# caidao22/pnode

Measured on AMD Instinct MI355X. Metric: time-steps/sec (fwd+adjoint), higher is better.
Workload: dtype f32; 1 GPU; C3a: MLP dynamics 3x512 tanh, batch 4096 x state_dim 512 per GPU, rk4 fixed h=0.01, 100 time steps, adjoint on, stages stored in HBM; batch_per_gpu=4096, state_elements_per_gpu=2097152, rejected_attempts=0, launch_mode=graph(auto), graph_revalidate_every=100, linear_param_grads=engine (8 of 8 parameter tensors; fused dW + db MFMA kernel on 4 layers), stage_tapes_retained=True, tunableop=False, parallelism=batch-sharded x1, one RCCL all-reduce of dL/dtheta per backward

## Files before the change

include/pnode_amd.h:

```cpp
#ifndef PNODE_AMD_H
#define PNODE_AMD_H

#include <stdint.h>

#ifdef __cplusplus
extern "C" {
#endif

#define PN_MAX_STAGES 7
#define PN_MAX_TERMS 8
#define PN_WGRAD_MAX_PAIRS 8
#define PN_WGRAD_EXACT_FP32 1
#define PN_WGRAD_TILE_64 2
#define PN_ABI_VERSION 4

typedef enum { PN_F32 = 0, PN_F64 = 1 } pn_dtype;

const char *pn_last_error(void);
int pn_abi_version(void);

typedef struct {
  int s;
  int order;
  int fsal;
// ... 46 lines not shown
int pn_colsum_accum_multi(void *stream, int dtype, int nsrc, const int64_t *rows, const int64_t *cols, const void *const *g,
                          void *const *mu, const double *alpha, void *work);
int64_t pn_colsum_work_bytes(int nsrc, const int64_t *rows, const int64_t *cols);
int pn_colsum_accum(void *stream, int dtype, int64_t rows, int64_t cols, const void *g, void *mu, double alpha, void *work);

typedef struct {
  const void *g, *x;
  void *pw, *pb;
  double alpha;
  int64_t out_f, in_f;
} pn_wgrad_pair;
int pn_linear_wgrad_supported(int dtype, int64_t rows, int64_t out_f, int64_t in_f);
int64_t pn_linear_wgrad_work_bytes(int dtype, int64_t out_f, int64_t in_f, int64_t *bias_bytes);
int pn_linear_wgrad(void *stream, int dtype, int64_t rows, int64_t out_f, int64_t in_f, const void *g, const void *x, double alpha,
                    void *pw, void *pb);
int pn_linear_wgrad_group(void *stream, int dtype, int64_t rows, int npairs, const pn_wgrad_pair *pairs, int flags);
int pn_linear_wgrad_finish(void *stream, int dtype, int64_t out_f, int64_t in_f, void *pw, void *pb, void *mu_w, void *mu_b);

#define PN_ACT_IDENTITY 0
#define PN_ACT_TANH 1
int pn_linear_fwd_supported(int dtype, int64_t rows, int64_t out_f, int64_t in_f);
int pn_linear_fwd(void *stream, int dtype, int64_t rows, int64_t out_f, int64_t in_f, const void *x, const void *w, const void *b, int act,
                  void *y);

int pn_linear_bwd_supported(int dtype, int64_t rows, int64_t out_f, int64_t in_f);
int pn_linear_bwd(void *stream, int dtype, int64_t rows, int64_t out_f, int64_t in_f, const void *g, const void *a, const void *w, void *gz,
                  void *dx);

int pn_dots(void *stream, int dtype, int64_t n, const void *x, int nk, const void *const *y,
            void *work, double *result_dev);
int64_t pn_dots_work_bytes(int64_t n);
int pn_lincomb(void *stream, int dtype, int64_t n, void *out, int nin, const void *const *x, const double *c);
int pn_stream_wait_scalars(void *stream, const double *host_ptr, int count, double *values);

int pn_copy(void *stream, int dtype, int64_t n, void *y, const void *x);
int pn_zero(void *stream, int dtype, int64_t n, void *y);

typedef enum { PN_K_STAGE = 0, PN_K_COMBINE_WRMS, PN_K_ADJ_THETA, PN_K_ADJ_ACCUM,
               PN_K_PARAM_ACCUM, PN_K_COPY, PN_K_DOTS, PN_K_LINCOMB, PN_K_LINEAR_WGRAD, PN_K_COUNT } pn_kernel_id;
int pn_prof_enable(int on);
int pn_prof_is_enabled(void);
int pn_tune_set(const char *spec);
int pn_prof_collect(int count, int64_t *launches, double *usec, double *bytes);
const char *pn_kernel_name(int kernel_id);

typedef struct pn_ts pn_ts;

pn_ts *pn_ts_create(void);
void pn_ts_destroy(pn_ts *ts);
int pn_ts_set_rk_type(pn_ts *ts, const char *rk_type);
// ... 160 lines not shown
```

pnode_amd/_lib.py:

```python
import ctypes
import os

import torch

_HERE = os.path.dirname(os.path.abspath(__file__))
LIB_PATH = os.path.join(_HERE, "lib", "libpnode_amd.so")

PN_MAX_STAGES = 7
PN_MAX_TERMS = 8
PN_F32, PN_F64 = 0, 1
PN_TRAJ_ALL, PN_TRAJ_SOLUTION, PN_TRAJ_BUDGET = 0, 1, 2
KERNEL_IDS = ("pn_rk_stage", "pn_rk_combine_wrms", "pn_adj_theta", "pn_adj_accum", "pn_param_accum", "pn_copy", "pn_dots", "pn_lincomb",
              "pn_linear_wgrad")


class PnError(RuntimeError):
    """A C-ABI entry point returned non-zero (stands where petsc4py.PETSc.Error did)."""


class Tableau(ctypes.Structure):
    _fields_ = [
        ("s", ctypes.c_int), ("order", ctypes.c_int), ("fsal", ctypes.c_int), ("has_embed", ctypes.c_int),
        ("A", (ctypes.c_double * PN_MAX_STAGES) * PN_MAX_STAGES),
        ("b", ctypes.c_double * PN_MAX_STAGES),
        ("bembed", ctypes.c_double * PN_MAX_STAGES),
        ("c", ctypes.c_double * PN_MAX_STAGES),
    ]


class WgradPair(ctypes.Structure):
    _fields_ = [("g", ctypes.c_void_p), ("x", ctypes.c_void_p), ("pw", ctypes.c_void_p), ("pb", ctypes.c_void_p),
                ("alpha", ctypes.c_double), ("out_f", ctypes.c_int64), ("in_f", ctypes.c_int64)]


PN_WGRAD_MAX_PAIRS = 8
PN_WGRAD_EXACT_FP32 = 1
PN_WGRAD_TILE_64 = 2
PN_ACT_IDENTITY, PN_ACT_TANH = 0, 1
PN_ABI_VERSION = 4
PN_DENSE_MAX_POW = 4
PN_DENSE_CHUNK = 32
PN_DENSE_NONTEMPORAL = 1
PN_ROWS_T, PN_ROWS_H, PN_ROWS_TFIRST, PN_ROWS_CACHED, PN_ROWS_ND = 0, 1, 2, 3, 4
PN_ROWS_SPANCTR, PN_ROWS_STEPS, PN_ROWS_REJ, PN_ROWS_REJ_STEP, PN_ROWS_PREV_REJ, PN_ROWS_FINISHED, PN_ROWS_FAIL, PN_ROWS_NI = 0, 1, 2, 3, 4, 5, 6, 8
_vp, _i, _i64, _d, _cp = ctypes.c_void_p, ctypes.c_int, ctypes.c_int64, ctypes.c_double, ctypes.c_char_p
_pd, _pi, _pi64 = ctypes.POINTER(ctypes.c_double), ctypes.POINTER(ctypes.c_int), ctypes.POINTER(ctypes.c_int64)
_pvp = ctypes.POINTER(ctypes.c_void_p)

STAGE_CB = ctypes.CFUNCTYPE(ctypes.c_int64, ctypes.c_void_p, ctypes.c_int, ctypes.c_double)
VJP_CB = ctypes.CFUNCTYPE(ctypes.c_int64, ctypes.c_void_p, ctypes.c_int, ctypes.c_double, ctypes.c_int, ctypes.c_double)
RK_STAGE_FN = ctypes.CFUNCTYPE(_i, _vp, _i, _i64, _vp, _vp, _i, _pvp, _pd)
RK_COMBINE_WRMS_FN = ctypes.CFUNCTYPE(_i, _vp, _i, _i64, _vp, _vp, _i, _pvp, _pd, _pd, _d, _d, _vp, _vp)
ADJ_THETA_FN = ctypes.CFUNCTYPE(_i, _vp, _i, _i64, _vp, _vp, _d, _i, _pvp, _pd)
ADJ_ACCUM_FN = ctypes.CFUNCTYPE(_i, _vp, _i, _i64, _vp, _vp, _i, _pvp, _pd, _vp, _vp, _d)


class VecOps(ctypes.Structure):
    _fields_ = [("rk_stage", RK_STAGE_FN), ("rk_combine_wrms", RK_COMBINE_WRMS_FN), ("adj_theta", ADJ_THETA_FN),
                ("adj_accum", ADJ_ACCUM_FN)]


# ... 46 lines not shown
    "pn_stream_wait_winf": (_i, [_vp, _vp, _i64, _pd]),
    "pn_winf_finish": (_i, [_vp, _i64, _pd]),
    "pn_pinned_scalar": (_i, [ctypes.POINTER(_vp), ctypes.POINTER(_vp)]),
    "pn_pinned_free": (_i, [_vp]),
    "pn_stream_create": (_i, [_i, ctypes.POINTER(_vp)]),
    "pn_stream_destroy": (_i, [_vp]),
    "pn_pinned_block": (_i, [_i64, ctypes.POINTER(_vp), ctypes.POINTER(_vp)]),
    "pn_stream_wait_scalar": (_i, [_vp, _vp, _pd]),
    "pn_adj_theta": (_i, [_vp, _i, _i64, _vp, _vp, _d, _i, _pvp, _pd]),
    "pn_adj_accum": (_i, [_vp, _i, _i64, _vp, _vp, _i, _pvp, _pd, _vp, _vp, _d]),
    "pn_param_accum": (_i, [_vp, _i, _vp, _d, _i, _pvp, _pi64, _pi64]),
    "pn_param_accum_multi": (_i, [_vp, _i, _vp, _i, _pd, _i, _pvp, _pi64, _pi64]),
    "pn_lincomb": (_i, [_vp, _i, _i64, _vp, _i, _pvp, _pd]),
    "pn_dots": (_i, [_vp, _i, _i64, _vp, _i, _pvp, _vp, _vp]),
    "pn_dots_work_bytes": (_i64, [_i64]),
    "pn_stream_wait_scalars": (_i, [_vp, _vp, _i, _pd]),
    "pn_linear_wgrad_supported": (_i, [_i, _i64, _i64, _i64]),
    "pn_linear_wgrad_work_bytes": (_i64, [_i, _i64, _i64, _pi64]),
    "pn_linear_wgrad": (_i, [_vp, _i, _i64, _i64, _i64, _vp, _vp, _d, _vp, _vp]),
    "pn_linear_wgrad_group": (_i, [_vp, _i, _i64, _i, ctypes.POINTER(WgradPair), _i]),
    "pn_linear_wgrad_finish": (_i, [_vp, _i, _i64, _i64, _vp, _vp, _vp, _vp]),
    "pn_linear_fwd_supported": (_i, [_i, _i64, _i64, _i64]),
    "pn_linear_fwd": (_i, [_vp, _i, _i64, _i64, _i64, _vp, _vp, _vp, _i, _vp]),
    "pn_linear_bwd_supported": (_i, [_i, _i64, _i64, _i64]),
    "pn_linear_bwd": (_i, [_vp, _i, _i64, _i64, _i64, _vp, _vp, _vp, _vp, _vp]),
    "pn_colsum_accum": (_i, [_vp, _i, _i64, _i64, _vp, _vp, _d, _vp]),
    "pn_colsum_accum_multi": (_i, [_vp, _i, _i, _pi64, _pi64, ctypes.POINTER(_vp), ctypes.POINTER(_vp), _pd, _vp]),
    "pn_colsum_work_bytes": (_i64, [_i, _pi64, _pi64]),
    "pn_copy": (_i, [_vp, _i, _i64, _vp, _vp]),
    "pn_zero": (_i, [_vp, _i, _i64, _vp]),
    "pn_prof_enable": (_i, [_i]),
    "pn_prof_is_enabled": (_i, []),
    "pn_tune_set": (_i, [_cp]),
    "pn_prof_collect": (_i, [_i, _pi64, _pd, _pd]),
    "pn_kernel_name": (_cp, [_i]),
    "pn_ts_create": (_vp, []),
    "pn_ts_destroy": (None, [_vp]),
    "pn_ts_set_rk_type": (_i, [_vp, _cp]),
    "pn_ts_get_tableau": (_i, [_vp, ctypes.POINTER(Tableau)]),
    "pn_ts_set_option": (_i, [_vp, _cp, _cp]),
    "pn_ts_wnorm_infinity": (_i, [_vp]),
    "pn_ts_is_adaptive": (_i, [_vp]),
    "pn_ts_set_scheme": (_i, [_vp, _i, _i]),
    "pn_ts_get_tolerances": (_i, [_vp, _pd, _pd]),
    "pn_ts_begin": (_i, [_vp, _d, _d, _i, _pd]),
    "pn_ts_attempt": (_i, [_vp, _pd, _pd]),
    "pn_ts_judge": (_i, [_vp, _d, _pi, _pi, _pi]),
    "pn_ts_count_fixed_steps": (_i64, [_vp]),
# ... 91 lines not shown
```

pnode_amd/_rk_sweep.py:

```python
import contextlib
import ctypes
import warnings

import torch

from . import _lib, options
from ._lib import PnError, check


def _mem_now(device):
    try:
        st = torch._C._cuda_memoryStats(device.index if device.index is not None else torch.cuda.current_device())
        return st["allocated_bytes"]["all"]["current"], st["reserved_bytes"]["all"]["current"]
    except Exception:
        return torch.cuda.memory_allocated(device), torch.cuda.memory_reserved(device)


class _RKState(object):
    __slots__ = "save T times full solution sol traj keep_tape tape_budget tape_steps tape_fsal K_fsal pingpong pp cur cur_slot ctl finished".split()


class RKSweep(object):
    def _func_with_grad(self, t, y, which="EX"):
        fn, params, names = ((self.funcIM, self._paramsI, self._pnamesI) if which == "IM"
# ... 694 lines not shown
            self._ops.wgrad_flags = (_lib.PN_WGRAD_EXACT_FP32 if exact else 0) | (_lib.PN_WGRAD_TILE_64 if tile64 else 0)
        self._setup_linear_fwd()
        sig = (id(self.funcEX), on, self._stepper_kind in (None, "imex"), tuple(id(p) for p in self._paramsE), gemm, side_on, exact, tile64)
        if sig == self._lin_sig:
            return
        self._lin_sig = sig
        if self._lin is not None:
            self._lin.remove()
            self._lin = None
        if on and sig[2] and self._paramsE:
            from ._lineargrad import LinearParamGrads
            lin = LinearParamGrads(self)
            lin.fused = not gemm
            lin.side_on = side_on
            lin.side_priority = side != "same-priority"
            if lin.install(self.funcEX, self._paramsE, self._poffE if self._stepper_kind == "imex" else self._poff):
                self._lin = lin

    def _setup_linear_fwd(self):
        mode = str(options.get_all().get("pn_linear_fwd", "auto"))
        mode = "auto" if mode == "auto" else ("1" if options.truthy(mode, False) else "0")
        bwd = str(options.get_all().get("pn_linear_bwd", "auto"))
        bwd = "auto" if bwd == "auto" else ("1" if options.truthy(bwd, False) else "0")
        from ._linearfwd import LinearFwd
        on = mode != "0" and self._stepper_kind in (None, "imex") and self.device.type == LinearFwd.device_type \
            and self.tensor_dtype == torch.float32 and hasattr(self._ops, "linear_fwd")
        sig = (id(self.funcEX), mode, on, tuple(id(p) for p in self._paramsE), bwd)
        if sig == self._fwd_sig:
            return
        self._fwd_sig = sig
        self._fwd = None
        if on and self._paramsE:
            fwd = LinearFwd(self)
            if fwd.install(self.funcEX, self._paramsE, mode, bwd):
                self._fwd = fwd

    @property
    def linear_fwd(self):
        fwd = self._fwd
        if fwd is None:
            return "stock modules (no eligible pair, not an fp32 state on a HIP device, a theta stepper, or -pn_linear_fwd 0)"
        if fwd.disabled:
            return "stock modules (%s)" % fwd.why
        return "fused (%d pairs, %d calls so far)" % (sum(len(p) for _, p in fwd.plans), fwd.n_fused)

    @property
    def linear_bwd(self):
        fwd = self._fwd
        if fwd is None or fwd.disabled:
            return "torch operations (the pairs run the stock modules: see linear_fwd)"
# ... 256 lines not shown
```

pnode_amd/_vecops.py:

```python
import contextlib
import ctypes
import warnings

import torch
import torch.nn as nn

from . import _lib, options
from ._lib import PnError, check


class HipVecOps(object):

    def __init__(self, device, dtype, n):
        if device.type != "cuda":
            raise RuntimeError(
                "pnode_amd runs on MI355X HIP devices only (got a %s tensor); there is no CPU path" % device.type)
        self.lib = _lib.load()
        self.device, self.dtype, self.n = device, dtype, n
        self.code = _lib.dtype_code(dtype)
        self.work = None
        self.dots_work = None
        self._err_host = self._err_dev = None
        self._pinned_stream = None
        self._seg_cache = {}
# ... 151 lines not shown
        self.linear_wgrad_group([(g, x, alpha, pw, pb)])

    MAX_WGRAD_PAIRS = _lib.PN_WGRAD_MAX_PAIRS

    wgrad_flags = 0

    def linear_wgrad_group(self, items, stream=None):
        st = self.stream() if stream is None else stream
        for k in range(0, len(items), self.MAX_WGRAD_PAIRS):
            part = items[k:k + self.MAX_WGRAD_PAIRS]
            arr = (_lib.WgradPair * len(part))()
            for q, (g, x, alpha, pw, pb) in zip(arr, part):
                q.g, q.x, q.pw, q.pb = g.data_ptr(), x.data_ptr(), pw.data_ptr(), (None if pb is None else pb.data_ptr())
                q.alpha, q.out_f, q.in_f = alpha, g.shape[1], x.shape[1]
            check(self.lib.pn_linear_wgrad_group(st, self.code, part[0][0].shape[0], len(part), arr, self.wgrad_flags))

    def linear_wgrad_finish(self, out_f, in_f, pw, pb, mu_w, mu_b):
        check(self.lib.pn_linear_wgrad_finish(self.stream(), self.code, out_f, in_f, pw.data_ptr(), None if pb is None else pb.data_ptr(),
                                              mu_w.data_ptr(), None if mu_b is None else mu_b.data_ptr()))

    def linear_fwd_supported(self, rows, out_f, in_f):
        return bool(self.lib.pn_linear_fwd_supported(self.code, rows, out_f, in_f))

    def linear_fwd(self, x, w, b, tanh, y=None):
        rows, in_f = x.shape
        out_f = w.shape[0]
        for v in (x, w, b, y):
            if v is not None and not (v.is_contiguous() and v.dtype == torch.float32 and v.device == x.device and x.is_cuda):
                raise PnError("pn_linear_fwd: contiguous fp32 tensors on one HIP device")
        if w.shape[1] != in_f or (b is not None and b.numel() != out_f):
            raise PnError("pn_linear_fwd: x (rows, in_f), w (out_f, in_f), b (out_f,)")
        if y is None:
            y = torch.empty((rows, out_f), dtype=x.dtype, device=x.device)
        elif tuple(y.shape) != (rows, out_f):
            raise PnError("pn_linear_fwd: y (rows, out_f)")
        check(self.lib.pn_linear_fwd(self.stream(), _lib.dtype_code(x.dtype), rows, out_f, in_f, x.data_ptr(), w.data_ptr(),
                                     None if b is None else b.data_ptr(), _lib.PN_ACT_TANH if tanh else _lib.PN_ACT_IDENTITY, y.data_ptr()))
        return y

    def linear_bwd_supported(self, rows, out_f, in_f):
        return bool(self.lib.pn_linear_bwd_supported(self.code, rows, out_f, in_f))

    def linear_bwd(self, g, a, w, gz=None, dx=None):
        rows, out_f = g.shape
        in_f = w.shape[1]
        for v in (g, a, w, gz, dx):
            if v is not None and not (v.is_contiguous() and v.dtype == torch.float32 and v.device == g.device and g.is_cuda):
                raise PnError("pn_linear_bwd: contiguous fp32 tensors on one HIP device")
        if tuple(a.shape) != (rows, out_f) or w.shape[0] != out_f:
            raise PnError("pn_linear_bwd: g and a (rows, out_f), w (out_f, in_f)")
        if gz is None:
            gz = torch.empty((rows, out_f), dtype=g.dtype, device=g.device)
        elif tuple(gz.shape) != (rows, out_f):
            raise PnError("pn_linear_bwd: gz (rows, out_f)")
        if dx is None:
            dx = torch.empty((rows, in_f), dtype=g.dtype, device=g.device)
        elif tuple(dx.shape) != (rows, in_f):
            raise PnError("pn_linear_bwd: dx (rows, in_f)")
        check(self.lib.pn_linear_bwd(self.stream(), self.code, rows, out_f, in_f, g.data_ptr(), a.data_ptr(), w.data_ptr(), gz.data_ptr(),
                                     dx.data_ptr()))
        return gz, dx

    dense_flags = _lib.PN_DENSE_NONTEMPORAL

    def dense_eval(self, out, u, Ks, coefs):
        m, nk = len(coefs), len(Ks)
        c = (ctypes.c_double * (m * nk))(*[x for row in coefs for x in row])
        check(self.lib.pn_rk_dense_eval(self.stream(), self.code, self.n, u.data_ptr(), nk, (ctypes.c_void_p * nk)(*[k.data_ptr() for k in Ks]),
                                        m, c, out.data_ptr(), out.stride(0), self.dense_flags))

    def dense_adjoint(self, Ds, G, g, coefs, accumulate=False):
        m, nd = g.shape[0], len(Ds)
        c = (ctypes.c_double * max(m * nd, 1))(*[x for row in coefs for x in row])
        check(self.lib.pn_rk_dense_adjoint(self.stream(), self.code, self.n, m, g.data_ptr(), g.stride(0), nd, c,
                                           (ctypes.c_void_p * max(nd, 1))(*[d.data_ptr() for d in Ds]),
                                           None if G is None else G.data_ptr(), 1 if accumulate else 0))

    def _tgrad_work(self):
        w = getattr(self, "_tg_work", None)
        if w is None:
            w = self._tg_work = torch.zeros(self.lib.pn_tgrad_work_bytes(self.n) // 8, dtype=torch.float64, device=self.device)
        return w

# ... 214 lines not shown
```

pnode_amd/csrc/pn_linear.hip:

```cpp
#include <hip/hip_runtime.h>

#include <cstdint>
#include <string>
#include <type_traits>

#include "pn_launch.h"
#include "pnode_amd.h"

namespace {

typedef float f32x16 __attribute__((ext_vector_type(16)));
typedef float f32x4 __attribute__((ext_vector_type(4)));
typedef double f64x4 __attribute__((ext_vector_type(4)));
typedef double f64x2 __attribute__((ext_vector_type(2)));

constexpr int kSplit = 8;
constexpr int BM = 64, BN = 64;
constexpr int kThreads = 512;
constexpr int kMaxPairs = PN_WGRAD_MAX_PAIRS;
constexpr int64_t kMaxWeights = (int64_t)1 << 22;

template <typename T>
struct Shape {
  static constexpr int BK = 32;
// ... 519 lines not shown
  for (int e = 0; e < VEC; ++e) z[e] = (T)0;
#pragma unroll
  for (int s = 0; s < kSplit; ++s) *reinterpret_cast<vec_t *>(PW + (size_t)s * mn + i) = z;
}

template <typename T>
__global__ __launch_bounds__(256) void pn_linear_bgrad_finish_kernel(double *__restrict__ PB, int M, int parts, T *__restrict__ mu) {
  const int m = blockIdx.x * 256 + threadIdx.x;
  if (m >= M) return;
  double s = 0.0;
  int k = 0;
  for (; k + 8 <= parts; k += 8) {
    double v[8];
#pragma unroll
    for (int j = 0; j < 8; ++j) v[j] = PB[(size_t)(k + j) * M + m];
#pragma unroll
    for (int j = 0; j < 8; ++j) s += v[j];
  }
  for (; k < parts; ++k) s += PB[(size_t)k * M + m];
  mu[m] += (T)s;
  for (k = 0; k < parts; ++k) PB[(size_t)k * M + m] = 0.0;
}

constexpr int FM = 64, FN = 128, FK = 32, kFwdThreads = 512;

struct FwdArgs {
  const float *x, *w, *b;
  float *y;
  int rows, out_f, in_f, act, ntn;
};

template <bool RAGGED>
__device__ __forceinline__ void linear_fwd_body(const FwdArgs &a) {
  constexpr int ROWB = 2 * FK, XPART = FM * ROWB, WPART = FN * ROWB, BUF = 3 * XPART + 3 * WPART;
  __shared__ __attribute__((aligned(16))) char smem[2 * BUF];
  const float *__restrict__ X = a.x;
  const float *__restrict__ W = a.w;
  const int rows = a.rows, out_f = a.out_f, in_f = a.in_f, ntn = a.ntn;
  const int nblk = (int)gridDim.x, bid = (int)blockIdx.x;
  const int tile = nblk % 8 == 0 ? (bid & 7) * (nblk >> 3) + (bid >> 3) : bid;
  const int tm = tile / ntn, tn = tile % ntn;
  const int t = threadIdx.x, lane = t & 63, w = t >> 6;
  const int kh = w >> 2, wm = w & 1, wn = (w >> 1) & 1;
  const int lrow = t >> 3, lc = t & 7;
  const int nslab = in_f / FK;
  const bool xok = !RAGGED || tm * FM + lrow < rows;
  const bool wok0 = !RAGGED || tn * FN + lrow < out_f, wok1 = !RAGGED || tn * FN + 64 + lrow < out_f;
  const float *xp = X + (size_t)(tm * FM + lrow) * in_f + lc * 4;
  const float *wp0 = W + (size_t)(tn * FN + lrow) * in_f + lc * 4;
  const float *wp1 = wp0 + (size_t)64 * in_f;
  const f32x4 zero4 = {0.f, 0.f, 0.f, 0.f};
  f32x4 xv, wv0, wv1;
  f32x16 acc0, acc1;
#pragma unroll
  for (int e = 0; e < 16; ++e) acc0[e] = 0.f, acc1[e] = 0.f;

  auto gload = [&](int slab) {
    xv = xok ? *reinterpret_cast<const f32x4 *>(xp + slab * FK) : zero4;
// ... 10 lines not shown
  auto lstore = [&](int buf) {
    char *b = smem + buf * BUF;
    split_store(xv, b, XPART);
    split_store(wv0, b + 3 * XPART, WPART);
    split_store(wv1, b + 3 * XPART + 64 * ROWB, WPART);
  };
  auto frag = [&](const char *part, int r0) -> s16x8 {
    const int row = r0 + (lane & 31);
    return *reinterpret_cast<const s16x8 *>(part + row * ROWB + (swz_row(row, 2 * kh + (lane >> 5)) << 4));
  };
  auto compute = [&](int buf) {
    const char *xb = smem + buf * BUF, *wb = xb + 3 * XPART;
    const s16x8 ah = frag(xb, wm * 32), am = frag(xb + XPART, wm * 32), al = frag(xb + 2 * XPART, wm * 32);
    {
      const s16x8 bh = frag(wb, wn * 64), bm = frag(wb + WPART, wn * 64), bl = frag(wb + 2 * WPART, wn * 64);
      six_products(acc0, ah, am, al, bh, bm, bl);
    }
    {
      const s16x8 bh = frag(wb, wn * 64 + 32), bm = frag(wb + WPART, wn * 64 + 32), bl = frag(wb + 2 * WPART, wn * 64 + 32);
      six_products(acc1, ah, am, al, bh, bm, bl);
    }
  };

  gload(0);
  lstore(0);
  if (nslab > 1) gload(1);
  __syncthreads();
  for (int s = 0; s < nslab; ++s) {
    if (s + 1 < nslab) lstore((s + 1) & 1);
    compute(s & 1);
    if (s + 2 < nslab) gload(s + 2);
    __syncthreads();
  }
  float(*red)[64] = reinterpret_cast<float(*)[64]>(smem);
  static_assert(sizeof(smem) >= 8 * 16 * 64 * sizeof(float), "the exchange is staged in the slab buffers");
#pragma unroll
  for (int e = 0; e < 16; ++e) red[w * 16 + e][lane] = kh == 0 ? acc1[e] : acc0[e];
  __syncthreads();
  const int col = tn * FN + wn * 64 + kh * 32 + (lane & 31);
  const bool colok = !RAGGED || col < out_f;
  const float bias = (a.b != nullptr && colok) ? a.b[col] : 0.f;
  const int row0 = tm * FM + wm * 32 + 4 * (lane >> 5);
  float *yp = a.y + (size_t)row0 * out_f + col;
  const bool tanh_act = a.act == PN_ACT_TANH;
#pragma unroll
  for (int e = 0; e < 16; ++e) {
    const float other = red[(w ^ 4) * 16 + e][lane];
    const float first = kh == 0 ? acc0[e] : other, second = kh == 0 ? other : acc1[e];
    float z = (first + second) + bias;
    if (tanh_act) z = tanhf(z);
    const int r = (e & 3) + 8 * (e >> 2);
    if (colok && (!RAGGED || row0 + r < rows)) yp[(size_t)r * out_f] = z;
  }
}

__global__ __launch_bounds__(kFwdThreads, 4) void pn_linear_fwd_kernel_f32x3(FwdArgs a) { linear_fwd_body<false>(a); }
__global__ __launch_bounds__(kFwdThreads, 4) void pn_linear_fwd_kernel_f32x3_ragged(FwdArgs a) { linear_fwd_body<true>(a); }

struct BwdArgs {
  const float *g, *a, *w;
  float *gz, *dx;
  int rows, out_f, in_f, ntn;
};

template <bool RAGGED>
__device__ __forceinline__ void linear_bwd_body(const BwdArgs &q) {
  constexpr int AROWB = 2 * FK, APART = FM * AROWB;
  constexpr int WROWB = 128, WIMG = FK * WROWB, WPART = 2 * WIMG;
  constexpr int BUF = 3 * APART + 3 * WPART;
  __shared__ __attribute__((aligned(16))) char smem[2 * BUF];
  const float *__restrict__ G = q.g;
  const float *__restrict__ A = q.a;
  const float *__restrict__ W = q.w;
  const int rows = q.rows, out_f = q.out_f, in_f = q.in_f, ntn = q.ntn;
  const int nblk = (int)gridDim.x, bid = (int)blockIdx.x;
  const int tile = nblk % 8 == 0 ? (bid & 7) * (nblk >> 3) + (bid >> 3) : bid;
  const int tm = tile / ntn, tn = tile % ntn;
  const int t = threadIdx.x, lane = t & 63, w = t >> 6;
  const int kh = w >> 2, wm = w & 1, wn = (w >> 1) & 1;
  const int lrow = t >> 3, lc = t & 7;
  const int krow = t >> 5, sub = (t >> 4) & 1, kc = t & 15;
  const int nslab = out_f / FK;
  const bool aok = !RAGGED || tm * FM + lrow < rows;
  const bool wok = !RAGGED || tn * FN + sub * 64 + kc * 4 < in_f;
  const bool keep = tn == 0 && aok;
  const size_t aoff = (size_t)(tm * FM + lrow) * out_f + lc * 4;
  const float *wp = W + (size_t)krow * in_f + tn * FN + sub * 64 + kc * 4;
  const f32x4 zero4 = {0.f, 0.f, 0.f, 0.f};
  f32x4 gv, av, wv0, wv1;
  f32x16 acc0, acc1;
#pragma unroll
  for (int e = 0; e < 16; ++e) acc0[e] = 0.f, acc1[e] = 0.f;

// ... 30 lines not shown
    s16x4 r[2];
#pragma unroll
    for (int u = 0; u < 2; ++u) {
      const int k = kh * 16 + 8 * (g4 >> 1) + 4 * u + q4;
      const int c = col0 + (g4 & 1) * 16 + 4 * p4;
      r[u] = __builtin_amdgcn_ds_read_tr16_b64_v4i16((__attribute__((address_space(3))) s16x4 *)(img + k * WROWB + swz_tr(k, c) * 2));
    }
    const s16x8 f = {r[0][0], r[0][1], r[0][2], r[0][3], r[1][0], r[1][1], r[1][2], r[1][3]};
    return f;
  };
  auto compute = [&](int buf) {
    const char *ab = smem + buf * BUF, *wb = ab + 3 * APART + wn * WIMG;
    const s16x8 ah = afrag(ab, wm * 32), am = afrag(ab + APART, wm * 32), al = afrag(ab + 2 * APART, wm * 32);
    {
      const s16x8 bh = wfrag(wb, 0), bm = wfrag(wb + WPART, 0), bl = wfrag(wb + 2 * WPART, 0);
      six_products(acc0, ah, am, al, bh, bm, bl);
    }
    {
      const s16x8 bh = wfrag(wb, 32), bm = wfrag(wb + WPART, 32), bl = wfrag(wb + 2 * WPART, 32);
      six_products(acc1, ah, am, al, bh, bm, bl);
    }
  };

  gload(0);
  lstore(0, 0);
  if (nslab > 1) gload(1);
  __syncthreads();
  for (int s = 0; s < nslab; ++s) {
    if (s + 1 < nslab) lstore(s + 1, (s + 1) & 1);
    compute(s & 1);
    if (s + 2 < nslab) gload(s + 2);
    __syncthreads();
  }
  float(*red)[64] = reinterpret_cast<float(*)[64]>(smem);
  static_assert(sizeof(smem) >= 8 * 16 * 64 * sizeof(float), "the exchange is staged in the slab buffers");
#pragma unroll
  for (int e = 0; e < 16; ++e) red[w * 16 + e][lane] = kh == 0 ? acc1[e] : acc0[e];
  __syncthreads();
  const int col = tn * FN + wn * 64 + kh * 32 + (lane & 31);
  const bool colok = !RAGGED || col < in_f;
  const int row0 = tm * FM + wm * 32 + 4 * (lane >> 5);
  float *dp = q.dx + (size_t)row0 * in_f + col;
#pragma unroll
  for (int e = 0; e < 16; ++e) {
    const float other = red[(w ^ 4) * 16 + e][lane];
    const float first = kh == 0 ? acc0[e] : other, second = kh == 0 ? other : acc1[e];
    const int r = (e & 3) + 8 * (e >> 2);
    if (colok && (!RAGGED || row0 + r < rows)) dp[(size_t)r * in_f] = first + second;
  }
}

__global__ __launch_bounds__(kFwdThreads, 4) void pn_linear_bwd_kernel_f32x3(BwdArgs a) { linear_bwd_body<false>(a); }
__global__ __launch_bounds__(kFwdThreads, 4) void pn_linear_bwd_kernel_f32x3_ragged(BwdArgs a) { linear_bwd_body<true>(a); }

int cu_count() {
  static int n = 0;
  if (n == 0) {
    int dev = 0, v = 0;
    if (hipGetDevice(&dev) == hipSuccess && hipDeviceGetAttribute(&v, hipDeviceAttributeMultiprocessorCount, dev) == hipSuccess && v > 0)
      n = v;
    else
      n = 256;
  }
  return n;
}

template <typename T>
int finish_t(hipStream_t st, int64_t out_f, int64_t in_f, void *pw, void *pb, void *mu_w, void *mu_b) {
  const size_t mn = (size_t)out_f * (size_t)in_f;
  constexpr int VEC = 16 / (int)sizeof(T);
  const char *name = "pn_linear_wgrad_finish";
  int rc = pn::launch(name, pn_linear_wgrad_finish_kernel<T>, dim3((unsigned)((mn / VEC + 255) / 256)), dim3(256), st, (T *)pw, mn, (T *)mu_w);
  if (!rc && pb != nullptr && mu_b != nullptr)
    rc = pn::launch(name, pn_linear_bgrad_finish_kernel<T>, dim3((unsigned)((out_f + 255) / 256)), dim3(256), st, (double *)pb, (int)out_f,
                    (int)(kSplit * (in_f / BN)), (T *)mu_b);
  return rc;
// ... 62 lines not shown

int pn_linear_wgrad(void *stream, int dtype, int64_t rows, int64_t out_f, int64_t in_f, const void *g, const void *x, double alpha,
                    void *pw, void *pb) {
  pn_wgrad_pair q;
  q.g = g, q.x = x, q.pw = pw, q.pb = pb, q.alpha = alpha, q.out_f = out_f, q.in_f = in_f;
  return pn_linear_wgrad_group(stream, dtype, rows, 1, &q, 0);
}

int pn_linear_wgrad_finish(void *stream, int dtype, int64_t out_f, int64_t in_f, void *pw, void *pb, void *mu_w, void *mu_b) {
  if (dtype != PN_F32 && dtype != PN_F64) return pn::fail("pn_linear_wgrad_finish: fp32 or fp64");
  if (!pn::aligned16(pw, mu_w)) return pn::fail("pn_linear_wgrad_finish: operands must be 16-byte aligned");
  return pn::with_dtype(dtype, [&](auto t) { return finish_t<decltype(t)>((hipStream_t)stream, out_f, in_f, pw, pb, mu_w, mu_b); });
}

int pn_linear_fwd_supported(int dtype, int64_t rows, int64_t out_f, int64_t in_f) {
  if (dtype != PN_F32) return 0;
  const int64_t lim = (int64_t)1 << 30;
  if (!(rows >= 256 && rows < lim && out_f > 0 && out_f < lim && out_f % 64 == 0 && in_f > 0 && in_f < lim && in_f % 64 == 0)) return 0;
  return ((rows + FM - 1) / FM) * ((out_f + FN - 1) / FN) < lim ? 1 : 0;
}

int pn_linear_fwd(void *stream, int dtype, int64_t rows, int64_t out_f, int64_t in_f, const void *x, const void *w, const void *b, int act,
                  void *y) {
  if (!pn_linear_fwd_supported(dtype, rows, out_f, in_f)) return pn::fail("pn_linear_fwd: unsupported dtype or shape (see pn_linear_fwd_supported)");
  if (act != PN_ACT_IDENTITY && act != PN_ACT_TANH) return pn::fail("pn_linear_fwd: act is PN_ACT_IDENTITY or PN_ACT_TANH");
  if (x == nullptr || w == nullptr || y == nullptr) return pn::fail("pn_linear_fwd: null operand");
  if (!pn::aligned16(x, w, y) || (reinterpret_cast<uintptr_t>(b) & 3)) return pn::fail("pn_linear_fwd: operands must be 16-byte aligned");
  if (x == y) return pn::fail("pn_linear_fwd: y must not be x (other workgroups still read the rows a workgroup writes)");
  FwdArgs a;
  a.x = (const float *)x, a.w = (const float *)w, a.b = (const float *)b, a.y = (float *)y;
  a.rows = (int)rows, a.out_f = (int)out_f, a.in_f = (int)in_f, a.act = act;
  a.ntn = (int)((out_f + FN - 1) / FN);
  const unsigned blocks = (unsigned)((rows + FM - 1) / FM) * (unsigned)a.ntn;
  const bool ragged = rows % FM != 0 || out_f % FN != 0;
  return pn::launch("pn_linear_fwd", ragged ? pn_linear_fwd_kernel_f32x3_ragged : pn_linear_fwd_kernel_f32x3, dim3(blocks), dim3(kFwdThreads),
                    (hipStream_t)stream, a);
}

int pn_linear_bwd_supported(int dtype, int64_t rows, int64_t out_f, int64_t in_f) {
  if (dtype != PN_F32) return 0;
  const int64_t lim = (int64_t)1 << 30;
  if (!(rows >= 256 && rows < lim && out_f > 0 && out_f < lim && out_f % 64 == 0 && in_f > 0 && in_f < lim && in_f % 64 == 0)) return 0;
  return ((rows + FM - 1) / FM) * ((in_f + FN - 1) / FN) < lim ? 1 : 0;
}

int pn_linear_bwd(void *stream, int dtype, int64_t rows, int64_t out_f, int64_t in_f, const void *g, const void *a, const void *w, void *gz,
                  void *dx) {
  if (!pn_linear_bwd_supported(dtype, rows, out_f, in_f)) return pn::fail("pn_linear_bwd: unsupported dtype or shape (see pn_linear_bwd_supported)");
  if (g == nullptr || a == nullptr || w == nullptr || gz == nullptr || dx == nullptr) return pn::fail("pn_linear_bwd: null operand");
  if (!pn::aligned16(g, a, w, gz, dx)) return pn::fail("pn_linear_bwd: operands must be 16-byte aligned");
  const size_t nz = (size_t)rows * (size_t)out_f * sizeof(float), nw = (size_t)out_f * (size_t)in_f * sizeof(float),
               nx = (size_t)rows * (size_t)in_f * sizeof(float);
  auto overlap = [](const void *p, size_t np, const void *r, size_t nr) {
    const uintptr_t p0 = reinterpret_cast<uintptr_t>(p), r0 = reinterpret_cast<uintptr_t>(r);
    return p0 < r0 + nr && r0 < p0 + np;
  };
  if (overlap(gz, nz, g, nz) || overlap(gz, nz, a, nz) || overlap(gz, nz, w, nw))
    return pn::fail("pn_linear_bwd: gz must not alias g, a or w (other workgroups still read them)");
  if (overlap(dx, nx, g, nz) || overlap(dx, nx, a, nz) || overlap(dx, nx, w, nw) || overlap(dx, nx, gz, nz))
    return pn::fail("pn_linear_bwd: dx must not alias g, a, w or gz");
  BwdArgs q;
  q.g = (const float *)g, q.a = (const float *)a, q.w = (const float *)w, q.gz = (float *)gz, q.dx = (float *)dx;
  q.rows = (int)rows, q.out_f = (int)out_f, q.in_f = (int)in_f;
  q.ntn = (int)((in_f + FN - 1) / FN);
  const unsigned blocks = (unsigned)((rows + FM - 1) / FM) * (unsigned)q.ntn;
  const bool ragged = rows % FM != 0 || in_f % FN != 0;
  return pn::launch("pn_linear_bwd", ragged ? pn_linear_bwd_kernel_f32x3_ragged : pn_linear_bwd_kernel_f32x3, dim3(blocks), dim3(kFwdThreads),
                    (hipStream_t)stream, q);
}

}
```

pnode_amd/options.py:

```python
import os
import shlex

_DB = {}


def _is_key(tok):
    if not tok.startswith("-") or len(tok) < 2:
        return False
    try:
        float(tok)
        return False
    except ValueError:
        return True


def parse(argv):
    out = {}
    toks = list(argv)
    i = 0
    while i < len(toks):
        tok = toks[i]
        if _is_key(tok):
            key = tok.lstrip("-")
            if i + 1 < len(toks) and not _is_key(toks[i + 1]):
# ... 20 lines not shown
def set_option(key, value=""):
    _DB[key.lstrip("-")] = "" if value is None else str(value)


def del_option(key):
    _DB.pop(key.lstrip("-"), None)


def clear():
    _DB.clear()


def get_all():
    return dict(_DB)


def truthy(value, default=True):
    if value is None:
        return default
    v = str(value).strip().lower()
    if v == "":
        return True
    return v in ("1", "true", "yes", "on")
```

Measured before the change: 1049 time-steps/s.

## Add triple-buffered software-pipelined MFMA loop for linear fwd and bwd kernels

Adds a pipelined slab loop for the f32x3 linear forward and backward kernels. It uses three LDS buffers, register-prefetches global loads two slabs ahead, double-buffers MFMA fragments, and interleaves instructions with sched_group_barrier hints. The pipelined kernel becomes the default for non-ragged shapes, and a -pn_linear_form plain option restores the old loop. The aim is to hide global and LDS latency behind MFMA work, at the cost of 1.5x the LDS use and a launch bound cut from 4 to 2, which reduces occupancy.

```diff
diff --git a/include/pnode_amd.h b/include/pnode_amd.h
--- a/include/pnode_amd.h
+++ b/include/pnode_amd.h
@@ -92,10 +92,15 @@
 int pn_linear_fwd_supported(int dtype, int64_t rows, int64_t out_f, int64_t in_f);
 int pn_linear_fwd(void *stream, int dtype, int64_t rows, int64_t out_f, int64_t in_f, const void *x, const void *w, const void *b, int act,
                   void *y);
+#define PN_LINEAR_FORM_PLAIN 1
+int pn_linear_fwd_form(void *stream, int dtype, int64_t rows, int64_t out_f, int64_t in_f, const void *x, const void *w, const void *b,
+                       int act, void *y, int flags);
 
 int pn_linear_bwd_supported(int dtype, int64_t rows, int64_t out_f, int64_t in_f);
 int pn_linear_bwd(void *stream, int dtype, int64_t rows, int64_t out_f, int64_t in_f, const void *g, const void *a, const void *w, void *gz,
                   void *dx);
+int pn_linear_bwd_form(void *stream, int dtype, int64_t rows, int64_t out_f, int64_t in_f, const void *g, const void *a, const void *w,
+                       void *gz, void *dx, int flags);
 
 int pn_dots(void *stream, int dtype, int64_t n, const void *x, int nk, const void *const *y,
             void *work, double *result_dev);
diff --git a/pnode_amd/_lib.py b/pnode_amd/_lib.py
--- a/pnode_amd/_lib.py
+++ b/pnode_amd/_lib.py
@@ -37,6 +37,7 @@
 PN_WGRAD_EXACT_FP32 = 1
 PN_WGRAD_TILE_64 = 2
 PN_ACT_IDENTITY, PN_ACT_TANH = 0, 1
+PN_LINEAR_FORM_PLAIN = 1
 PN_ABI_VERSION = 4
 PN_DENSE_MAX_POW = 4
 PN_DENSE_CHUNK = 32
@@ -129,8 +130,10 @@
     "pn_linear_wgrad_finish": (_i, [_vp, _i, _i64, _i64, _vp, _vp, _vp, _vp]),
     "pn_linear_fwd_supported": (_i, [_i, _i64, _i64, _i64]),
     "pn_linear_fwd": (_i, [_vp, _i, _i64, _i64, _i64, _vp, _vp, _vp, _i, _vp]),
+    "pn_linear_fwd_form": (_i, [_vp, _i, _i64, _i64, _i64, _vp, _vp, _vp, _i, _vp, _i]),
     "pn_linear_bwd_supported": (_i, [_i, _i64, _i64, _i64]),
     "pn_linear_bwd": (_i, [_vp, _i, _i64, _i64, _i64, _vp, _vp, _vp, _vp, _vp]),
+    "pn_linear_bwd_form": (_i, [_vp, _i, _i64, _i64, _i64, _vp, _vp, _vp, _vp, _vp, _i]),
     "pn_colsum_accum": (_i, [_vp, _i, _i64, _i64, _vp, _vp, _d, _vp]),
     "pn_colsum_accum_multi": (_i, [_vp, _i, _i, _pi64, _pi64, ctypes.POINTER(_vp), ctypes.POINTER(_vp), _pd, _vp]),
     "pn_colsum_work_bytes": (_i64, [_i, _pi64, _pi64]),
diff --git a/pnode_amd/_rk_sweep.py b/pnode_amd/_rk_sweep.py
--- a/pnode_amd/_rk_sweep.py
+++ b/pnode_amd/_rk_sweep.py
@@ -740,10 +740,13 @@
         mode = "auto" if mode == "auto" else ("1" if options.truthy(mode, False) else "0")
         bwd = str(options.get_all().get("pn_linear_bwd", "auto"))
         bwd = "auto" if bwd == "auto" else ("1" if options.truthy(bwd, False) else "0")
+        form = options.linear_form()
+        if hasattr(self._ops, "linear_flags"):
+            self._ops.linear_flags = _lib.PN_LINEAR_FORM_PLAIN if form == "plain" else 0
         from ._linearfwd import LinearFwd
         on = mode != "0" and self._stepper_kind in (None, "imex") and self.device.type == LinearFwd.device_type \
             and self.tensor_dtype == torch.float32 and hasattr(self._ops, "linear_fwd")
-        sig = (id(self.funcEX), mode, on, tuple(id(p) for p in self._paramsE), bwd)
+        sig = (id(self.funcEX), mode, on, tuple(id(p) for p in self._paramsE), bwd, form)
         if sig == self._fwd_sig:
             return
         self._fwd_sig = sig
diff --git a/pnode_amd/_vecops.py b/pnode_amd/_vecops.py
--- a/pnode_amd/_vecops.py
+++ b/pnode_amd/_vecops.py
@@ -197,7 +197,9 @@
     def linear_fwd_supported(self, rows, out_f, in_f):
         return bool(self.lib.pn_linear_fwd_supported(self.code, rows, out_f, in_f))
 
-    def linear_fwd(self, x, w, b, tanh, y=None):
+    linear_flags = 0
+
+    def linear_fwd(self, x, w, b, tanh, y=None, flags=None):
         rows, in_f = x.shape
         out_f = w.shape[0]
         for v in (x, w, b, y):
@@ -209,14 +211,15 @@
             y = torch.empty((rows, out_f), dtype=x.dtype, device=x.device)
         elif tuple(y.shape) != (rows, out_f):
             raise PnError("pn_linear_fwd: y (rows, out_f)")
-        check(self.lib.pn_linear_fwd(self.stream(), _lib.dtype_code(x.dtype), rows, out_f, in_f, x.data_ptr(), w.data_ptr(),
-                                     None if b is None else b.data_ptr(), _lib.PN_ACT_TANH if tanh else _lib.PN_ACT_IDENTITY, y.data_ptr()))
+        check(self.lib.pn_linear_fwd_form(self.stream(), _lib.dtype_code(x.dtype), rows, out_f, in_f, x.data_ptr(), w.data_ptr(),
+                                          None if b is None else b.data_ptr(), _lib.PN_ACT_TANH if tanh else _lib.PN_ACT_IDENTITY, y.data_ptr(),
+                                          self.linear_flags if flags is None else flags))
         return y
 
     def linear_bwd_supported(self, rows, out_f, in_f):
         return bool(self.lib.pn_linear_bwd_supported(self.code, rows, out_f, in_f))
 
-    def linear_bwd(self, g, a, w, gz=None, dx=None):
+    def linear_bwd(self, g, a, w, gz=None, dx=None, flags=None):
         rows, out_f = g.shape
         in_f = w.shape[1]
         for v in (g, a, w, gz, dx):
@@ -232,8 +235,8 @@
             dx = torch.empty((rows, in_f), dtype=g.dtype, device=g.device)
         elif tuple(dx.shape) != (rows, in_f):
             raise PnError("pn_linear_bwd: dx (rows, in_f)")
-        check(self.lib.pn_linear_bwd(self.stream(), self.code, rows, out_f, in_f, g.data_ptr(), a.data_ptr(), w.data_ptr(), gz.data_ptr(),
-                                     dx.data_ptr()))
+        check(self.lib.pn_linear_bwd_form(self.stream(), self.code, rows, out_f, in_f, g.data_ptr(), a.data_ptr(), w.data_ptr(), gz.data_ptr(),
+                                          dx.data_ptr(), self.linear_flags if flags is None else flags))
         return gz, dx
 
     dense_flags = _lib.PN_DENSE_NONTEMPORAL
diff --git a/pnode_amd/csrc/pn_linear.hip b/pnode_amd/csrc/pn_linear.hip
--- a/pnode_amd/csrc/pn_linear.hip
+++ b/pnode_amd/csrc/pn_linear.hip
@@ -565,6 +565,72 @@
   for (k = 0; k < parts; ++k) PB[(size_t)k * M + m] = 0.0;
 }
 
+struct Frags {
+  s16x8 ah, am, al, b0h, b0m, b0l, b1h, b1m, b1l;
+};
+
+template <int I, int NREAD, int RPG, bool RD, bool ST>
+__device__ __forceinline__ void pipe_groups() {
+  if constexpr (I < 12) {
+    __builtin_amdgcn_sched_group_barrier(0x008, 1, 0);
+    constexpr int left = NREAD - I * RPG, nr = left < 0 ? 0 : (left < RPG ? left : RPG);
+    if constexpr (ST) __builtin_amdgcn_sched_group_barrier(0x002, 8, 0);
+    if constexpr (RD && nr > 0) __builtin_amdgcn_sched_group_barrier(0x100, nr, 0);
+    if constexpr (ST) {
+      if constexpr (I >= 3 && (I & 1)) __builtin_amdgcn_sched_group_barrier(0x200, 1, 0);
+    }
+    pipe_groups<I + 1, NREAD, RPG, RD, ST>();
+  }
+}
+
+template <int NREAD, int NLOAD, typename G, typename GL, typename LS, typename RF>
+__device__ __forceinline__ void pipelined_slabs(const int nslab, const int BUF, f32x16 &acc0, f32x16 &acc1, GL gload, LS lstore, RF read) {
+  constexpr int RPG = NREAD > 12 ? 2 : 1;
+  G g0, g1;
+  Frags f0, f1;
+  int rb = BUF, wb = 2 * BUF, fb = 0;
+  auto step = [&](auto ld, auto rd, auto st, const Frags &cur, Frags &nxt, const G &gcur, G &gnxt, int s) {
+    constexpr bool LD = decltype(ld)::value, RD = decltype(rd)::value, ST = decltype(st)::value;
+    if constexpr (LD) gload(gnxt, s + 3);
+    if constexpr (RD) read(nxt, rb);
+    if constexpr (ST) lstore(gcur, s + 2, wb);
+    six_products(acc0, cur.ah, cur.am, cur.al, cur.b0h, cur.b0m, cur.b0l);
+    six_products(acc1, cur.ah, cur.am, cur.al, cur.b1h, cur.b1m, cur.b1l);
+    if constexpr (LD) {
+      __builtin_amdgcn_sched_group_barrier(0x002, 2 * NLOAD, 0);
+      __builtin_amdgcn_sched_group_barrier(0x020, NLOAD, 0);
+    }
+    pipe_groups<0, NREAD, RPG, RD, ST>();
+    __builtin_amdgcn_sched_barrier(0);
+    __syncthreads();
+    __builtin_amdgcn_sched_barrier(0);
+    const int r = rb;
+    rb = wb, wb = fb, fb = r;
+  };
+  constexpr std::true_type yes{};
+  constexpr std::false_type no{};
+  gload(g0, 0);
+  gload(g1, 1);
+  lstore(g0, 0, 0);
+  if (nslab > 2) gload(g0, 2);
+  lstore(g1, 1, BUF);
+  __syncthreads();
+  read(f0, 0);
+  __builtin_amdgcn_sched_barrier(0);
+  int s = 0;
+  for (; s + 4 < nslab; s += 2) {
+    step(yes, yes, yes, f0, f1, g0, g1, s);
+    step(yes, yes, yes, f1, f0, g1, g0, s + 1);
+  }
+  if (nslab >= 4) {
+    step(yes, yes, yes, f0, f1, g0, g1, s);
+    step(no, yes, yes, f1, f0, g1, g0, s + 1);
+    s += 2;
+  }
+  step(no, yes, no, f0, f1, g0, g1, s);
+  step(no, no, no, f1, f0, g1, g0, s + 1);
+}
+
 constexpr int FM = 64, FN = 128, FK = 32, kFwdThreads = 512;
 
 struct FwdArgs {
@@ -573,10 +639,15 @@
   int rows, out_f, in_f, act, ntn;
 };
 
-template <bool RAGGED>
+struct FwdLoads {
+  f32x4 x, w0, w1;
+};
+
+template <bool RAGGED, bool PIPE>
 __device__ __forceinline__ void linear_fwd_body(const FwdArgs &a) {
+  static_assert(!(RAGGED && PIPE), "the pipelined loop loads without tests");
   constexpr int ROWB = 2 * FK, XPART = FM * ROWB, WPART = FN * ROWB, BUF = 3 * XPART + 3 * WPART;
-  __shared__ __attribute__((aligned(16))) char smem[2 * BUF];
+  __shared__ __attribute__((aligned(16))) char smem[(PIPE ? 3 : 2) * BUF];
   const float *__restrict__ X = a.x;
   const float *__restrict__ W = a.w;
   const int rows = a.rows, out_f = a.out_f, in_f = a.in_f, ntn = a.ntn;
@@ -633,15 +704,37 @@
     }
   };
 
-  gload(0);
-  lstore(0);
-  if (nslab > 1) gload(1);
-  __syncthreads();
-  for (int s = 0; s < nslab; ++s) {
-    if (s + 1 < nslab) lstore((s + 1) & 1);
-    compute(s & 1);
-    if (s + 2 < nslab) gload(s + 2);
+  if constexpr (PIPE) {
+    pipelined_slabs<9, 3, FwdLoads>(
+        nslab, BUF, acc0, acc1,
+        [&](FwdLoads &g, int slab) {
+          g.x = *reinterpret_cast<const f32x4 *>(xp + slab * FK);
+          g.w0 = *reinterpret_cast<const f32x4 *>(wp0 + slab * FK);
+          g.w1 = *reinterpret_cast<const f32x4 *>(wp1 + slab * FK);
+        },
+        [&](const FwdLoads &g, int, int boff) {
+          char *b = smem + boff;
+          split_store(g.x, b, XPART);
+          split_store(g.w0, b + 3 * XPART, WPART);
+          split_store(g.w1, b + 3 * XPART + 64 * ROWB, WPART);
+        },
+        [&](Frags &f, int boff) {
+          const char *xb = smem + boff, *wb = xb + 3 * XPART;
+          f.ah = frag(xb, wm * 32), f.am = frag(xb + XPART, wm * 32), f.al = frag(xb + 2 * XPART, wm * 32);
+          f.b0h = frag(wb, wn * 64), f.b0m = frag(wb + WPART, wn * 64), f.b0l = frag(wb + 2 * WPART, wn * 64);
+          f.b1h = frag(wb, wn * 64 + 32), f.b1m = frag(wb + WPART, wn * 64 + 32), f.b1l = frag(wb + 2 * WPART, wn * 64 + 32);
+        });
+  } else {
+    gload(0);
+    lstore(0);
+    if (nslab > 1) gload(1);
     __syncthreads();
+    for (int s = 0; s < nslab; ++s) {
+      if (s + 1 < nslab) lstore((s + 1) & 1);
+      compute(s & 1);
+      if (s + 2 < nslab) gload(s + 2);
+      __syncthreads();
+    }
   }
   float(*red)[64] = reinterpret_cast<float(*)[64]>(smem);
   static_assert(sizeof(smem) >= 8 * 16 * 64 * sizeof(float), "the exchange is staged in the slab buffers");
@@ -665,8 +758,9 @@
   }
 }
 
-__global__ __launch_bounds__(kFwdThreads, 4) void pn_linear_fwd_kernel_f32x3(FwdArgs a) { linear_fwd_body<false>(a); }
-__global__ __launch_bounds__(kFwdThreads, 4) void pn_linear_fwd_kernel_f32x3_ragged(FwdArgs a) { linear_fwd_body<true>(a); }
+__global__ __launch_bounds__(kFwdThreads, 4) void pn_linear_fwd_kernel_f32x3(FwdArgs a) { linear_fwd_body<false, false>(a); }
+__global__ __launch_bounds__(kFwdThreads, 4) void pn_linear_fwd_kernel_f32x3_ragged(FwdArgs a) { linear_fwd_body<true, false>(a); }
+__global__ __launch_bounds__(kFwdThreads, 2) void pn_linear_fwd_kernel_f32x3_pipe(FwdArgs a) { linear_fwd_body<false, true>(a); }
 
 struct BwdArgs {
   const float *g, *a, *w;
@@ -674,12 +768,17 @@
   int rows, out_f, in_f, ntn;
 };
 
-template <bool RAGGED>
+struct BwdLoads {
+  f32x4 g, a, w0, w1;
+};
+
+template <bool RAGGED, bool PIPE>
 __device__ __forceinline__ void linear_bwd_body(const BwdArgs &q) {
+  static_assert(!(RAGGED && PIPE), "the pipelined loop loads without tests");
   constexpr int AROWB = 2 * FK, APART = FM * AROWB;
   constexpr int WROWB = 128, WIMG = FK * WROWB, WPART = 2 * WIMG;
   constexpr int BUF = 3 * APART + 3 * WPART;
-  __shared__ __attribute__((aligned(16))) char smem[2 * BUF];
+  __shared__ __attribute__((aligned(16))) char smem[(PIPE ? 3 : 2) * BUF];
   const float *__restrict__ G = q.g;
   const float *__restrict__ A = q.a;
   const float *__restrict__ W = q.w;
@@ -756,15 +855,52 @@
     }
   };
 
-  gload(0);
-  lstore(0, 0);
-  if (nslab > 1) gload(1);
-  __syncthreads();
-  for (int s = 0; s < nslab; ++s) {
-    if (s + 1 < nslab) lstore(s + 1, (s + 1) & 1);
-    compute(s & 1);
-    if (s + 2 < nslab) gload(s + 2);
+  if constexpr (PIPE) {
+    auto run = [&](auto keep_c) {
+      constexpr bool KEEP = decltype(keep_c)::value;
+      pipelined_slabs<15, 4, BwdLoads>(
+          nslab, BUF, acc0, acc1,
+          [&](BwdLoads &l, int slab) {
+            l.g = *reinterpret_cast<const f32x4 *>(G + aoff + slab * FK);
+            l.a = *reinterpret_cast<const f32x4 *>(A + aoff + slab * FK);
+            l.w0 = *reinterpret_cast<const f32x4 *>(wp + (size_t)(slab * FK) * in_f);
+            l.w1 = *reinterpret_cast<const f32x4 *>(wp + (size_t)(slab * FK + 16) * in_f);
+          },
+          [&](const BwdLoads &l, int slab, int boff) {
+            char *b = smem + boff;
+            f32x4 z;
+            {
+#pragma clang fp contract(off)
+#pragma unroll
+              for (int e = 0; e < 4; ++e) z[e] = l.g[e] * __builtin_fmaf(-l.a[e], l.a[e], 1.f);
+            }
+            if constexpr (KEEP) *reinterpret_cast<f32x4 *>(q.gz + aoff + slab * FK) = z;
+            split_store(z, b + aso, APART);
+            split_store(l.w0, b + 3 * APART + wso, WPART);
+            split_store(l.w1, b + 3 * APART + wso + 16 * WROWB, WPART);
+          },
+          [&](Frags &f, int boff) {
+            const char *ab = smem + boff, *wb = ab + 3 * APART + wn * WIMG;
+            f.ah = afrag(ab, wm * 32), f.am = afrag(ab + APART, wm * 32), f.al = afrag(ab + 2 * APART, wm * 32);
+            f.b0h = wfrag(wb, 0), f.b0m = wfrag(wb + WPART, 0), f.b0l = wfrag(wb + 2 * WPART, 0);
+            f.b1h = wfrag(wb, 32), f.b1m = wfrag(wb + WPART, 32), f.b1l = wfrag(wb + 2 * WPART, 32);
+          });
+    };
+    if (keep)
+      run(std::true_type{});
+    else
+      run(std::false_type{});
+  } else {
+    gload(0);
+    lstore(0, 0);
+    if (nslab > 1) gload(1);
     __syncthreads();
+    for (int s = 0; s < nslab; ++s) {
+      if (s + 1 < nslab) lstore(s + 1, (s + 1) & 1);
+      compute(s & 1);
+      if (s + 2 < nslab) gload(s + 2);
+      __syncthreads();
+    }
   }
   float(*red)[64] = reinterpret_cast<float(*)[64]>(smem);
   static_assert(sizeof(smem) >= 8 * 16 * 64 * sizeof(float), "the exchange is staged in the slab buffers");
@@ -784,8 +920,9 @@
   }
 }
 
-__global__ __launch_bounds__(kFwdThreads, 4) void pn_linear_bwd_kernel_f32x3(BwdArgs a) { linear_bwd_body<false>(a); }
-__global__ __launch_bounds__(kFwdThreads, 4) void pn_linear_bwd_kernel_f32x3_ragged(BwdArgs a) { linear_bwd_body<true>(a); }
+__global__ __launch_bounds__(kFwdThreads, 4) void pn_linear_bwd_kernel_f32x3(BwdArgs a) { linear_bwd_body<false, false>(a); }
+__global__ __launch_bounds__(kFwdThreads, 4) void pn_linear_bwd_kernel_f32x3_ragged(BwdArgs a) { linear_bwd_body<true, false>(a); }
+__global__ __launch_bounds__(kFwdThreads, 2) void pn_linear_bwd_kernel_f32x3_pipe(BwdArgs a) { linear_bwd_body<false, true>(a); }
 
 int cu_count() {
   static int n = 0;
@@ -894,6 +1031,12 @@
 
 int pn_linear_fwd(void *stream, int dtype, int64_t rows, int64_t out_f, int64_t in_f, const void *x, const void *w, const void *b, int act,
                   void *y) {
+  return pn_linear_fwd_form(stream, dtype, rows, out_f, in_f, x, w, b, act, y, 0);
+}
+
+int pn_linear_fwd_form(void *stream, int dtype, int64_t rows, int64_t out_f, int64_t in_f, const void *x, const void *w, const void *b,
+                       int act, void *y, int flags) {
+  if (flags & ~PN_LINEAR_FORM_PLAIN) return pn::fail("pn_linear_fwd_form: unknown flag (PN_LINEAR_FORM_PLAIN is the only one)");
   if (!pn_linear_fwd_supported(dtype, rows, out_f, in_f)) return pn::fail("pn_linear_fwd: unsupported dtype or shape (see pn_linear_fwd_supported)");
   if (act != PN_ACT_IDENTITY && act != PN_ACT_TANH) return pn::fail("pn_linear_fwd: act is PN_ACT_IDENTITY or PN_ACT_TANH");
   if (x == nullptr || w == nullptr || y == nullptr) return pn::fail("pn_linear_fwd: null operand");
@@ -905,8 +1048,8 @@
   a.ntn = (int)((out_f + FN - 1) / FN);
   const unsigned blocks = (unsigned)((rows + FM - 1) / FM) * (unsigned)a.ntn;
   const bool ragged = rows % FM != 0 || out_f % FN != 0;
-  return pn::launch("pn_linear_fwd", ragged ? pn_linear_fwd_kernel_f32x3_ragged : pn_linear_fwd_kernel_f32x3, dim3(blocks), dim3(kFwdThreads),
-                    (hipStream_t)stream, a);
+  auto kern = ragged ? pn_linear_fwd_kernel_f32x3_ragged : ((flags & PN_LINEAR_FORM_PLAIN) ? pn_linear_fwd_kernel_f32x3 : pn_linear_fwd_kernel_f32x3_pipe);
+  return pn::launch("pn_linear_fwd", kern, dim3(blocks), dim3(kFwdThreads), (hipStream_t)stream, a);
 }
 
 int pn_linear_bwd_supported(int dtype, int64_t rows, int64_t out_f, int64_t in_f) {
@@ -918,6 +1061,12 @@
 
 int pn_linear_bwd(void *stream, int dtype, int64_t rows, int64_t out_f, int64_t in_f, const void *g, const void *a, const void *w, void *gz,
                   void *dx) {
+  return pn_linear_bwd_form(stream, dtype, rows, out_f, in_f, g, a, w, gz, dx, 0);
+}
+
+int pn_linear_bwd_form(void *stream, int dtype, int64_t rows, int64_t out_f, int64_t in_f, const void *g, const void *a, const void *w,
+                       void *gz, void *dx, int flags) {
+  if (flags & ~PN_LINEAR_FORM_PLAIN) return pn::fail("pn_linear_bwd_form: unknown flag (PN_LINEAR_FORM_PLAIN is the only one)");
   if (!pn_linear_bwd_supported(dtype, rows, out_f, in_f)) return pn::fail("pn_linear_bwd: unsupported dtype or shape (see pn_linear_bwd_supported)");
   if (g == nullptr || a == nullptr || w == nullptr || gz == nullptr || dx == nullptr) return pn::fail("pn_linear_bwd: null operand");
   if (!pn::aligned16(g, a, w, gz, dx)) return pn::fail("pn_linear_bwd: operands must be 16-byte aligned");
@@ -937,8 +1086,8 @@
   q.ntn = (int)((in_f + FN - 1) / FN);
   const unsigned blocks = (unsigned)((rows + FM - 1) / FM) * (unsigned)q.ntn;
   const bool ragged = rows % FM != 0 || in_f % FN != 0;
-  return pn::launch("pn_linear_bwd", ragged ? pn_linear_bwd_kernel_f32x3_ragged : pn_linear_bwd_kernel_f32x3, dim3(blocks), dim3(kFwdThreads),
-                    (hipStream_t)stream, q);
-}
-
-}
+  auto kern = ragged ? pn_linear_bwd_kernel_f32x3_ragged : ((flags & PN_LINEAR_FORM_PLAIN) ? pn_linear_bwd_kernel_f32x3 : pn_linear_bwd_kernel_f32x3_pipe);
+  return pn::launch("pn_linear_bwd", kern, dim3(blocks), dim3(kFwdThreads), (hipStream_t)stream, q);
+}
+
+}
diff --git a/pnode_amd/options.py b/pnode_amd/options.py
--- a/pnode_amd/options.py
+++ b/pnode_amd/options.py
@@ -66,3 +66,10 @@
     if v == "":
         return True
     return v in ("1", "true", "yes", "on")
+
+
+def linear_form():
+    v = str(_DB.get("pn_linear_form", "auto")).strip().lower()
+    if v not in ("auto", "plain"):
+        raise ValueError("-pn_linear_form %r: auto or plain" % v)
+    return v
```

Result: faster. 1103 time-steps/s (median of 6 runs) (+5.1%).
